# thevasudevgupta/gsoc-wav2vec2

Hardware: AMD Instinct MI355X
Metric: audio-seconds/s (wav2vec2-base forward, 246000-sample pad) (higher is better)
Workload: dtype f32

## Files before the change

gsoc-wav2vec2_amd/csrc/common.h:

```cpp
#pragma once

#include <hip/hip_runtime.h>
#include <stdint.h>
#include <stdio.h>

#include <atomic>

#include <string>

#include "../../include/w2v2.h"

namespace w2v2 {

void set_error(const char* fmt, ...);

#define W2V2_HIP_CHECK(expr)                                                            \
    do {                                                                                \
        hipError_t _e = (expr);                                                         \
        if (_e != hipSuccess) {                                                         \
            ::w2v2::set_error("%s failed: %s (%s:%d)", #expr, hipGetErrorString(_e),    \
                              __FILE__, __LINE__);                                      \
            return W2V2_EHIP;                                                           \
        }                                                                               \
    } while (0)
// ... 98 lines not shown
    ~ProfScope() {
        if (--tl_prof_depth == 0) tl_launch_family = outer_family;
        if (tok >= 0) profiler_end(p, tok, s);
    }
};

extern thread_local Profiler* tl_step_prof;
struct StepProfScope {
    Profiler* outer;
    explicit StepProfScope(Profiler* p) : outer(tl_step_prof) { tl_step_prof = p; }
    ~StepProfScope() { tl_step_prof = outer; }
};

int launch_gemm(Profiler* prof, const float* A, int64_t lda, int64_t strideA, const float* B,
                int64_t ldb, float* C, int64_t ldc, int64_t strideC, const float* bias,
                const float* residual, int M, int N, int K, int nbatch, int act, hipStream_t s);

void gemm_f32_force_ring(int route);
bool gemm_f32_ring_ok(int tile, const float* A, int64_t lda, int64_t strideA, const float* B, int64_t ldb, int64_t strideB,
                      int M, int N, int K);
int launch_gemm_f32_ring(int tile, bool persist, const float* A, int64_t lda, int64_t strideA, const float* B, int64_t ldb,
                         int64_t strideB, float* C, int64_t ldc, int64_t strideC, const float* bias, const float* residual, int M,
                         int N, int K, int nbatch, int act, hipStream_t s);
int launch_gemm_f32_ring_split(bool persist, int64_t main_tiles, const float* A, int64_t lda, const float* B, int64_t ldb, float* C,
                               int64_t ldc, const float* bias, const float* residual, int M, int N, int K, int act, hipStream_t s);

int launch_gemm_bf16(Profiler* prof, const float* A, int64_t lda, int64_t strideA, const float* B, int64_t ldb,
                     int64_t strideB, float* C, int64_t ldc, int64_t strideC, const float* bias,
                     const float* residual, int M, int N, int K, int nbatch, int act, hipStream_t s);
bool gemm_split_supported(const float* A, int64_t lda, int64_t strideA, int M, int N, int K);
int launch_split_weight(const float* w, uint16_t* planes, int K, int N, hipStream_t s);
int launch_gemm_split(Profiler* prof, const float* A, int64_t lda, int64_t strideA, const uint16_t* planes, float* C, int64_t ldc,
                      int64_t strideC, const float* bias, const float* residual, int M, int N, int K, int nbatch, int act,
                      hipStream_t s);

bool gemm_split_sw_ok(const uint16_t* A16, int64_t planeA, int64_t lda, int64_t strideA, int M, int N, int K);
int launch_split_weight_sw(const float* w, uint16_t* img, int K, int N, int fmt, void* scratch, hipStream_t s);
int launch_split_planes(const float* x, uint16_t* planes, int64_t plane, int64_t n, int fmt, int* range_flag, hipStream_t s);
int launch_gemm_split_sw(Profiler* prof, int fmt, const uint16_t* A16, int64_t planeA, int64_t lda, int64_t strideA, const uint16_t* Bimg,
                         const float* out_scale, float* C, uint16_t* C16, int64_t planeC, int64_t ldc, int64_t strideC, const float* bias,
                         const float* residual, int M, int N, int K, int nbatch, int act, int* range_flag, hipStream_t s);

int launch_check_select_forms(unsigned long long* mismatches_dev , hipStream_t s);

struct GemmShadows {
    const uint16_t* A16 = nullptr;
    const uint16_t* B16 = nullptr;
    uint16_t* C16 = nullptr;
// ... 345 lines not shown
```

gsoc-wav2vec2_amd/csrc/gemm_f32.hip:

```cpp
#include <stdlib.h>


#include "common.h"
#include "gemm_epilogue.h"

namespace w2v2 {

using f32x16 = __attribute__((ext_vector_type(16))) float;
using f32x4 = __attribute__((ext_vector_type(4))) float;

namespace {

constexpr int BK = 32;
constexpr int LDA_S = BK + 4;

struct GemmArgs {
    const float* A;
    const float* B;
    float* C;
    const float* bias;
    const float* residual;
    int64_t lda, ldb, ldc, strideA, strideB, strideC;
    int M, N, K, act;
    int tiles_m, tiles_n;
// ... 326 lines not shown
        const int64_t e = i * 4, row = e / N;
        const int col = (int)(e % N);
        float4 acc = reinterpret_cast<const float4*>(slabs)[i];
        for (int z = 1; z < S; ++z) {
            const float4 v = reinterpret_cast<const float4*>(slabs + (int64_t)z * M * N)[i];
            acc.x += v.x; acc.y += v.y; acc.z += v.z; acc.w += v.w;
        }
        if (bias) { acc.x += bias[col]; acc.y += bias[col + 1]; acc.z += bias[col + 2]; acc.w += bias[col + 3]; }
        acc.x = apply_act(acc.x, act); acc.y = apply_act(acc.y, act); acc.z = apply_act(acc.z, act); acc.w = apply_act(acc.w, act);
        if (residual) {
            const float4 r = *reinterpret_cast<const float4*>(residual + row * ldc + col);
            acc.x += r.x; acc.y += r.y; acc.z += r.z; acc.w += r.w;
        }
        *reinterpret_cast<float4*>(C + row * ldc + col) = acc;
    }
}

thread_local int tl_precision = 0;
thread_local int tl_ring = -1;

constexpr int RING_DEFAULT = 2;
int ring_route() { return tl_ring >= 0 ? tl_ring : tune_int("W2V2_GEMM_RING", RING_DEFAULT); }

}

void gemm_set_precision(int mode) { tl_precision = mode; }
void gemm_f32_force_ring(int route) { tl_ring = route; }
int gemm_get_precision() { return tl_precision; }

int launch_gemm(Profiler* prof, const float* A, int64_t lda, int64_t strideA, const float* B,
                int64_t ldb, float* C, int64_t ldc, int64_t strideC, const float* bias,
                const float* residual, int M, int N, int K, int nbatch, int act, hipStream_t s) {
    return launch_gemm_ex(prof, A, lda, strideA, B, ldb, 0, C, ldc, strideC, bias, residual, M, N, K, nbatch, act, s);
}

int launch_gemm_ex(Profiler* prof, const float* A, int64_t lda, int64_t strideA, const float* B,
                   int64_t ldb, int64_t strideB, float* C, int64_t ldc, int64_t strideC, const float* bias,
                   const float* residual, int M, int N, int K, int nbatch, int act, hipStream_t s) {
    if (tl_precision == 1)
        return launch_gemm_bf16(prof, A, lda, strideA, B, ldb, strideB, C, ldc, strideC, bias, residual, M, N, K, nbatch, act, s);
    W2V2_REQUIRE(A && B && C, "gemm: null operand");
    W2V2_REQUIRE(M > 0 && N > 0 && K > 0 && nbatch > 0, "gemm: bad sizes M=%d N=%d K=%d batch=%d", M, N, K, nbatch);
    W2V2_REQUIRE(lda >= 1 && ldb >= N && ldc >= N && ldc < (1 << 23), "gemm: bad leading dimensions");
    W2V2_REQUIRE(act >= 0 && act <= 2, "gemm: bad activation %d", act);
    GemmArgs g;
    g.A = A; g.B = B; g.C = C; g.bias = bias; g.residual = residual;
    g.lda = lda; g.ldb = ldb; g.ldc = ldc; g.strideA = strideA; g.strideB = strideB; g.strideC = strideC;
    g.M = M; g.N = N; g.K = K; g.act = act;
    const bool fast = (K % BK == 0) && (N % 4 == 0) && (lda % 4 == 0) && (ldb % 4 == 0) &&
                      (strideA % 4 == 0) && (strideB % 4 == 0) && ((reinterpret_cast<uintptr_t>(A) & 15) == 0) &&
                      ((reinterpret_cast<uintptr_t>(B) & 15) == 0);
    ProfScope ps(prof, FAM_GEMM, 2.0 * M * (double)N * K * nbatch,
                 4.0 * nbatch * ((double)M * K + (double)M * N) + 4.0 * (double)K * N, s);
    int cfg = forced_cfg();
    const bool by_shape = cfg < 0;
    if (cfg < 0 && fast && nbatch == 1 && strideB == 0 && K >= 1024 && (ldc % 4) == 0 &&
        ((reinterpret_cast<uintptr_t>(C) | reinterpret_cast<uintptr_t>(residual) | reinterpret_cast<uintptr_t>(bias)) & 15) == 0) {
        const int64_t tiles64 = (int64_t)((M + 63) / 64) * ((N + 63) / 64);
        int S = 1;
        for (int cand = 8; cand >= 2; cand >>= 1)
            if (K % (cand * BK) == 0 && K / cand >= 256 && tiles64 * cand <= 512) { S = cand; break; }
        if (S > 1 && tiles64 <= 256) {
            const size_t need = (size_t)S * M * N;
// ... 2 lines not shown
            if (int e = stream_scratch(SCRATCH_SPLITK, s, need * sizeof(float), &raw)) return e;
            ws = reinterpret_cast<float*>(raw);
            GemmArgs h = g;
            h.C = ws; h.bias = nullptr; h.residual = nullptr; h.act = 0;
            h.K = K / S; h.strideA = K / S; h.strideB = (int64_t)(K / S) * ldb; h.ldc = N; h.strideC = (int64_t)M * N;
            if (int e = launch_dma<2, 2, 2, 32, 64, 64>(h, S, s)) return e;
            const int64_t n4 = (int64_t)M * N / 4;
            int64_t blocks = (n4 + 255) / 256;
            blocks = blocks > 2048 ? 2048 : blocks;
            W2V2_LAUNCH(splitk_reduce_kernel, dim3((unsigned)blocks), dim3(256), 0, s, ws, C, bias, residual, M, N, ldc, S, act);
            W2V2_HIP_CHECK(hipGetLastError());
            return W2V2_OK;
        }
    }
    if (cfg < 0) {
        cfg = 7;
        const int64_t tiles128 = (int64_t)((M + 127) / 128) * ((N + 127) / 128) * nbatch;
        if (fast && tiles128 < 384) cfg = 16;
        const int tail_knob = tune_int("W2V2_GEMM_TAIL", 1);
        const int64_t tn = (N + 127) / 128, S = 512, r = tiles128 % S;
        if (tail_knob && fast && cfg == 7 && nbatch == 1 && tiles128 > S && r != 0 && tune_int("W2V2_GEMM_TAIL_DIV", 4) * r <= S) {
            const int64_t main_rows = ((tiles128 - r) / tn) * 128;
            const int ring_flat = by_shape && tune_int("W2V2_GEMM_TAIL_FLAT", 1) ? ring_route() : 0;
            if (ring_flat && strideB == 0 && M % 128 == 0 && N % 128 == 0 && gemm_f32_ring_ok(1, A, lda, 0, B, ldb, 0, M, N, K) &&
                gemm_f32_ring_ok(2, A, lda, 0, B, ldb, 0, M, N, K))
                return launch_gemm_f32_ring_split(ring_flat == 2, tiles128 - r, A, lda, B, ldb, C, ldc, bias, residual, M, N, K, act, s);
            if (main_rows > 0 && main_rows < M) {
                GemmArgs h = g;
                h.M = (int)main_rows;
                const int ring = by_shape ? ring_route() : 0;
                if (ring && strideB == 0 && gemm_f32_ring_ok(1, A, lda, strideA, B, ldb, strideB, h.M, N, K)) {
                    if (int e = launch_gemm_f32_ring(1, ring == 2, A, lda, strideA, B, ldb, strideB, C, ldc, strideC, bias, residual,
                                                     h.M, N, K, 1, act, s))
                        return e;
                } else if (int e = launch_dma<2, 4, 2>(h, 1, s)) {
                    return e;
                }
                GemmArgs t = g;
                t.A = g.A + main_rows * lda;
                t.C = g.C + main_rows * ldc;
                t.residual = g.residual ? g.residual + main_rows * ldc : nullptr;
                t.M = M - (int)main_rows;
                if (ring && strideB == 0 && gemm_f32_ring_ok(2, t.A, lda, strideA, B, ldb, strideB, t.M, N, K))
                    return launch_gemm_f32_ring(2, ring == 2, t.A, lda, strideA, B, ldb, strideB, t.C, ldc, strideC, bias,
                                                t.residual, t.M, N, K, 1, act, s);
                return launch_dma<2, 2, 2, 32, 64, 64>(t, 1, s);
            }
        }
    }
    if (cfg == 16 && fast && by_shape) {
        const int ring = ring_route();
        if (ring && strideB == 0 && gemm_f32_ring_ok(2, A, lda, strideA, B, ldb, strideB, M, N, K))
            return launch_gemm_f32_ring(2, ring == 2, A, lda, strideA, B, ldb, strideB, C, ldc, strideC, bias, residual, M, N, K,
                                        nbatch, act, s);
    }
    const int wide_min = tune_int("W2V2_GEMM_WIDE", 1536);
    if (cfg == 7 && fast && wide_min > 0 && N % 128 == 0) {
        const int64_t tm256 = (M + 255) / 256, tiles256 = tm256 * (N / 128) * nbatch;
        if (tiles256 >= wide_min && (tm256 * 256 - M) * 40 <= M) {
            const int ring = by_shape ? ring_route() : 0;
            if (ring && strideB == 0 && gemm_f32_ring_ok(0, A, lda, strideA, B, ldb, strideB, M, N, K))
                return launch_gemm_f32_ring(0, ring == 2, A, lda, strideA, B, ldb, strideB, C, ldc, strideC, bias, residual, M, N, K,
                                            nbatch, act, s);
            return launch_dma<4, 2, 2, 16, 256, 128>(g, nbatch, s);
        }
    }
    if (cfg == 7 && fast) {
        const int ring = by_shape ? ring_route() : 0;
        if (ring && strideB == 0 && gemm_f32_ring_ok(1, A, lda, strideA, B, ldb, strideB, M, N, K))
            return launch_gemm_f32_ring(1, ring == 2, A, lda, strideA, B, ldb, strideB, C, ldc, strideC, bias, residual, M, N, K,
                                        nbatch, act, s);
    }
    switch (cfg) {
        case 16: if (fast) return launch_dma<2, 2, 2, 32, 64, 64>(g, nbatch, s); return launch_cfg<128, 128, 2, 2, 2>(g, fast, nbatch, s);
        case 14: if (fast) return launch_dma<2, 3, 2, 32, 128, 96>(g, nbatch, s); return launch_cfg<128, 128, 2, 2, 2>(g, fast, nbatch, s);
        case 1: return launch_cfg<128, 256, 2, 2, 1>(g, fast, nbatch, s);
        case 2: return launch_cfg<256, 128, 2, 2, 1>(g, fast, nbatch, s);
        case 3: return launch_cfg<256, 256, 4, 2, 2>(g, fast, nbatch, s);
        case 4: if (fast) return launch_dma<2, 2, 2>(g, nbatch, s); return launch_cfg<128, 128, 2, 2, 2>(g, fast, nbatch, s);
        case 6: if (fast) return launch_dma<4, 2, 2>(g, nbatch, s); return launch_cfg<128, 128, 2, 2, 2>(g, fast, nbatch, s);
        case 7: if (fast) return launch_dma<2, 4, 2>(g, nbatch, s); return launch_cfg<128, 128, 2, 2, 2>(g, fast, nbatch, s);
        case 9: if (fast) return launch_dma<2, 4, 3, 16>(g, nbatch, s); return launch_cfg<128, 128, 2, 2, 2>(g, fast, nbatch, s);
        case 10: if (fast) return launch_dma<2, 4, 4, 16>(g, nbatch, s); return launch_cfg<128, 128, 2, 2, 2>(g, fast, nbatch, s);
        case 11: if (fast) return launch_dma<2, 2, 4, 16>(g, nbatch, s); return launch_cfg<128, 128, 2, 2, 2>(g, fast, nbatch, s);
        case 12: if (fast && g.N >= 256) return launch_dma<4, 4, 1, 32, 256, 256>(g, nbatch, s); return launch_cfg<128, 128, 2, 2, 2>(g, fast, nbatch, s);
        case 13: if (fast && g.N >= 128) return launch_dma<4, 2, 1, 32, 256, 128>(g, nbatch, s); return launch_cfg<128, 128, 2, 2, 2>(g, fast, nbatch, s);
        case 8: if (fast) return launch_dma<4, 4, 1>(g, nbatch, s); return launch_cfg<128, 128, 2, 2, 2>(g, fast, nbatch, s);
#ifdef W2V2_TUNING
        case 17: if (fast && g.N >= 256) return launch_dma<2, 4, 2, 16, 128, 256>(g, nbatch, s); return launch_dma<2, 4, 2>(g, nbatch, s);
        case 18: if (fast && g.N >= 128) return launch_dma<4, 2, 2, 16, 256, 128>(g, nbatch, s); return launch_dma<2, 4, 2>(g, nbatch, s);
        case 19: if (fast && g.N >= 256) return launch_dma<2, 4, 2, 32, 128, 256>(g, nbatch, s); return launch_dma<2, 4, 2>(g, nbatch, s);
#endif
        default: return launch_cfg<128, 128, 2, 2, 2>(g, fast, nbatch, s);
    }
// ... 4 lines not shown
```

gsoc-wav2vec2_amd/csrc/gemm_f32_sw.hip:

```cpp
#include "common.h"
#include "gemm_epilogue.h"
#include "gemm_sw_common.h"

namespace w2v2 {

namespace {

struct GemmRingArgs {
    const float* A;
    const float* B;
    float* C;
    const float* bias;
    const float* residual;
    int64_t lda, ldb, ldc, strideA, strideB, strideC;
    int M, N, K, act;
    int tiles_m, tiles_n, nbatch;
    int gm;
    int total;
    int first;
};

template <int WM, int WN, int BKT, int BM, int BN, int NS>
struct RingCfg {
    static constexpr int STAGE = (BM * BKT + BKT * BN) * 4;
    static constexpr int LDS = NS * STAGE;
    static constexpr int NW = WM * WN;
    static constexpr int NPA = BM * BKT / 256, NPB = BKT * BN / 256;
    static constexpr int PPA = NPA / NW, PPB = NPB / NW;
    static constexpr int P = PPA + PPB;
    static_assert(NPA % NW == 0 && NPB % NW == 0, "every wave issues the same number of pieces (counted waits)");
    static_assert((NS - 2) * P <= 63, "vmcnt field");
};

template <int WM, int WN, int BKT, int BM, int BN, int NS, bool QUAD = false>
__global__ __launch_bounds__(WM* WN * 64) __attribute__((amdgpu_waves_per_eu(4))) void gemm_f32_ring_kernel(GemmRingArgs g) {
    using R_ = RingCfg<WM, WN, BKT, BM, BN, NS>;
    constexpr int NW = R_::NW, PPA = R_::PPA, PPB = R_::PPB, P = R_::P, STAGE = R_::STAGE;
    constexpr int RPP = 256 / BKT;
    constexpr int SPR = BKT / 4;
    constexpr int SW = BKT == 32 ? 1 : 2;
    constexpr int WTM = BM / WM, WTN = BN / WN, MT = WTM / 32, NTL = WTN / 32;
    extern __shared__ __attribute__((aligned(16))) float smem[];
    const int tid = threadIdx.x, lane = tid & 63, wave = __builtin_amdgcn_readfirstlane(tid >> 6);
    const int wm = wave / WN, wn = wave % WN, li = lane & 31, lh = lane >> 5;
    const unsigned lds0 = (unsigned)(uintptr_t)(__attribute__((address_space(3))) float*)smem;

    const int nwg = g.tiles_m * g.tiles_n, total = g.total, G = gridDim.x;
    const int ntl = (total - (int)blockIdx.x + G - 1) / G;
    const int nk = g.K / BKT, nsteps = ntl * nk;
    auto tile_of = [&](int i, int& z, int& m0, int& n0) {
        const int v = (int)blockIdx.x + i * G;
        const int q = total >> 3, r = total & 7, xcd = v & 7, idx = v >> 3;
        int t = (xcd < r ? xcd * (q + 1) : r * (q + 1) + (xcd - r) * q) + idx;
        int sub = 0;
        if constexpr (QUAD) {
            sub = t & 3;
            t = g.first + (t >> 2);
        }
        z = t / nwg;
        t -= z * nwg;
        int tm = t / g.tiles_n, tn = t % g.tiles_n;
        if (g.gm > 0) grouped_tile(t, g.tiles_m, g.tiles_n, g.gm, tm, tn);
        m0 = tm * BM;
        n0 = tn * BN;
        if constexpr (QUAD) {
            m0 = 2 * m0 + (sub >> 1) * BM;
            n0 = 2 * n0 + (sub & 1) * BN;
        }
    };

    int ii = 0, ikt = 0, ist = 0;
    const unsigned char* baseA = nullptr;
    const unsigned char* baseB = nullptr;
    uint32_t offA[PPA], offB[PPB];
    auto uniform_ptr = [](const void* p) {
        const uint64_t v = reinterpret_cast<uint64_t>(p);
        const uint32_t lo = __builtin_amdgcn_readfirstlane((uint32_t)v), hi = __builtin_amdgcn_readfirstlane((uint32_t)(v >> 32));
        return reinterpret_cast<const unsigned char*>(((uint64_t)hi << 32) | lo);
    };
    auto set_issue_tile = [&](int i) {
        int z, m0, n0;
        tile_of(i, z, m0, n0);
        baseA = uniform_ptr(g.A + (int64_t)z * g.strideA + (int64_t)m0 * g.lda);
        baseB = uniform_ptr(g.B + (int64_t)z * g.strideB + n0);
#pragma unroll
        for (int p = 0; p < PPA; ++p) {
            const int r = (wave + p * NW) * RPP + lane / SPR;
            const int rr = m0 + r < g.M ? r : g.M - 1 - m0;
// ... 82 lines not shown
            const bool more = s + NS - 1 < nsteps;
            if (more) issue_step();
            __builtin_amdgcn_sched_barrier(0);
            compute(cst);
            __builtin_amdgcn_sched_barrier(0);
            ring_barrier(more);
            cst = cst + 1 == NS ? 0 : cst + 1;
        }
        int z, m0, n0;
        tile_of(ci, z, m0, n0);
        const int64_t tile_off = (int64_t)z * g.strideC + (int64_t)(m0 + wm * WTM) * g.ldc + (n0 + wn * WTN);
        int act = g.act, ldc = (int)g.ldc, eli = li, elh = lh;
        const float* res = g.residual;
        const float* bias = g.bias;
        asm volatile("" : "+s"(act), "+s"(res), "+s"(bias), "+s"(ldc), "+v"(eli), "+v"(elh));
        __builtin_amdgcn_s_setprio(0);
        gemm_epilogue<MT, NTL, false>(acc, g.C + tile_off, nullptr, res ? res + tile_off : nullptr, bias ? bias + (n0 + wn * WTN) : nullptr,
                                     ldc, g.M - (m0 + wm * WTM), g.N - (n0 + wn * WTN), act, eli, elh);
        __builtin_amdgcn_s_setprio(1);
    }
    __builtin_amdgcn_s_setprio(0);
}

template <int WM, int WN, int BKT, int BM, int BN, int NS, bool QUAD = false>
int launch_ring(GemmRingArgs& g, bool persist, hipStream_t s, int64_t first = -1, int gm = 0) {
    using R_ = RingCfg<WM, WN, BKT, BM, BN, NS>;
    static_assert(2 * R_::LDS <= 160 * 1024, "two blocks per CU");
    constexpr int TM = QUAD ? 2 * BM : BM, TN = QUAD ? 2 * BN : BN;
    g.tiles_m = (g.M + TM - 1) / TM;
    g.tiles_n = (g.N + TN - 1) / TN;
    int64_t total = (int64_t)g.tiles_m * g.tiles_n * g.nbatch;
    W2V2_REQUIRE(first < 0 || (first > 0 && first < total && g.nbatch == 1 && g.M % TM == 0 && g.N % TN == 0), "gemm ring: bad split");
    W2V2_REQUIRE(!QUAD || first > 0, "gemm ring: quarter tiles need a split");
    g.first = QUAD ? (int)first : 0;
    if (first > 0) total = QUAD ? 4 * (total - first) : first;
    W2V2_REQUIRE(total < (1ll << 31), "gemm ring: %lld tiles", (long long)total);
    g.total = (int)total;
    constexpr int PER_CU = WM * WN == 8 ? 2 : 160 * 1024 / R_::LDS > 4 ? 4 : 160 * 1024 / R_::LDS;
    int grid = (int)total;
    if (persist) {
        int dev = 0, cus = 0;
        W2V2_HIP_CHECK(hipGetDevice(&dev));
        W2V2_HIP_CHECK(hipDeviceGetAttribute(&cus, hipDeviceAttributeMultiprocessorCount, dev));
        const int resident = (PER_CU * cus) & ~7;
        if (resident >= 8 && total > resident) grid = resident;
    }
    g.gm = first > 0 ? gm : g.nbatch == 1 ? tile_group_rows(g.tiles_m, g.tiles_n, (int64_t)BM * g.K * 4, BM == 256 ? 96 : 32 * PER_CU) : 0;
    static std::atomic<bool> attr_set{false};
    if (!attr_set) {
        W2V2_HIP_CHECK(hipFuncSetAttribute(reinterpret_cast<const void*>(gemm_f32_ring_kernel<WM, WN, BKT, BM, BN, NS, QUAD>),
                                           hipFuncAttributeMaxDynamicSharedMemorySize, R_::LDS));
        attr_set = true;
    }
    W2V2_LAUNCH((gemm_f32_ring_kernel<WM, WN, BKT, BM, BN, NS, QUAD>), dim3(grid), dim3(WM * WN * 64), R_::LDS, s, g);
    W2V2_HIP_CHECK(hipGetLastError());
    return W2V2_OK;
}

}

bool gemm_f32_ring_ok(int tile, const float* A, int64_t lda, int64_t strideA, const float* B, int64_t ldb, int64_t strideB,
                      int M, int N, int K) {
    const int BM = tile == 0 ? 256 : tile == 1 ? 128 : 64, BKT = tile == 2 ? 32 : 16;
    const bool align = ((reinterpret_cast<uintptr_t>(A) | reinterpret_cast<uintptr_t>(B)) & 15) == 0 && lda % 4 == 0 &&
                       ldb % 4 == 0 && strideA % 4 == 0 && strideB % 4 == 0;
    return align && K % BKT == 0 && N % 4 == 0 && N >= 4 && (int64_t)BM * lda * 4 < (1ll << 31) &&
           (int64_t)BKT * ldb * 4 < (1ll << 31) && M > 0;
}

int launch_gemm_f32_ring(int tile, bool persist, const float* A, int64_t lda, int64_t strideA, const float* B, int64_t ldb,
                         int64_t strideB, float* C, int64_t ldc, int64_t strideC, const float* bias, const float* residual, int M,
                         int N, int K, int nbatch, int act, hipStream_t s) {
    W2V2_REQUIRE(tile >= 0 && tile <= 2, "gemm ring: tile %d", tile);
    W2V2_REQUIRE(gemm_f32_ring_ok(tile, A, lda, strideA, B, ldb, strideB, M, N, K), "gemm ring: unsupported shape M=%d N=%d K=%d", M, N, K);
    GemmRingArgs g;
    g.A = A; g.B = B; g.C = C; g.bias = bias; g.residual = residual;
    g.lda = lda; g.ldb = ldb; g.ldc = ldc; g.strideA = strideA; g.strideB = strideB; g.strideC = strideC;
    g.M = M; g.N = N; g.K = K; g.act = act; g.nbatch = nbatch;
    if (tile == 0) return launch_ring<4, 2, 16, 256, 128, 3>(g, persist, s);
    if (tile == 1) return launch_ring<2, 4, 16, 128, 128, 4>(g, persist, s);
    return launch_ring<2, 2, 32, 64, 64, 3>(g, persist, s);
}

int launch_gemm_f32_ring_split(bool persist, int64_t main_tiles, const float* A, int64_t lda, const float* B, int64_t ldb, float* C,
                               int64_t ldc, const float* bias, const float* residual, int M, int N, int K, int act, hipStream_t s) {
    W2V2_REQUIRE(M % 128 == 0 && N % 128 == 0 && gemm_f32_ring_ok(1, A, lda, 0, B, ldb, 0, M, N, K) && gemm_f32_ring_ok(2, A, lda, 0, B, ldb, 0, M, N, K),
                 "gemm ring split: unsupported shape M=%d N=%d K=%d", M, N, K);
    GemmRingArgs g;
    g.A = A; g.B = B; g.C = C; g.bias = bias; g.residual = residual;
    g.lda = lda; g.ldb = ldb; g.ldc = ldc; g.strideA = 0; g.strideB = 0; g.strideC = 0;
    g.M = M; g.N = N; g.K = K; g.act = act; g.nbatch = 1;
    const int gm = tile_group_rows(M / 128, N / 128, (int64_t)128 * K * 4, 64);
    if (int e = launch_ring<2, 4, 16, 128, 128, 4>(g, persist, s, main_tiles, gm)) return e;
    return launch_ring<2, 2, 32, 64, 64, 3, true>(g, false, s, main_tiles, gm);
}

}
```

gsoc-wav2vec2_amd/csrc/w2v2_api.hip:

```cpp
#include <algorithm>
#include <mutex>
#include <atomic>
#include <stdarg.h>
#include <stdlib.h>
#include <string.h>

#include <map>
#include <string>
#include <unordered_map>
#include <vector>

#include "common.h"
#include "model.h"

namespace w2v2 {

static thread_local char g_err[1024] = "";
void set_error(const char* fmt, ...) {
    va_list ap;
    va_start(ap, fmt);
    vsnprintf(g_err, sizeof(g_err), fmt, ap);
    va_end(ap);
}

// ... 597 lines not shown
}
int w2v2_profile_reset(w2v2_model* m) {
    W2V2_REQUIRE(m, "profile_reset: null model");
    profiler_reset(m->prof);
    return W2V2_OK;
}

int w2v2_op_gemm(const float* A, int64_t lda, int64_t strideA, const float* B, int64_t ldb, float* C,
                 int64_t ldc, int64_t strideC, const float* bias, const float* residual, int32_t M,
                 int32_t N, int32_t K, int32_t nbatch, int32_t act, void* stream) {
    return launch_gemm(nullptr, A, lda, strideA, B, ldb, C, ldc, strideC, bias, residual, M, N, K, nbatch, act,
                       reinterpret_cast<hipStream_t>(stream));
}
int w2v2_op_gemm_variant(const float* A, int64_t lda, int64_t strideA, const float* B, int64_t ldb, float* C,
                         int64_t ldc, int64_t strideC, const float* bias, const float* residual, int32_t M,
                         int32_t N, int32_t K, int32_t nbatch, int32_t act, int32_t variant, void* stream) {
    W2V2_REQUIRE(variant >= -1 && variant <= 2, "op_gemm_variant: variant %d (-1 by shape, 0 double buffer, 1 ring, 2 persistent ring)", variant);
    gemm_f32_force_ring(variant);
    const int e = launch_gemm(nullptr, A, lda, strideA, B, ldb, C, ldc, strideC, bias, residual, M, N, K, nbatch, act,
                              reinterpret_cast<hipStream_t>(stream));
    gemm_f32_force_ring(-1);
    return e;
}
int w2v2_op_set_precision(int32_t mode) {
    W2V2_REQUIRE(mode >= W2V2_PRECISION_FP32 && mode <= W2V2_PRECISION_F16X2, "op_set_precision: unknown mode %d", mode);
    gemm_set_precision(mode);
    return W2V2_OK;
}
int w2v2_op_gemm_bf16(const float* A, int64_t lda, int64_t strideA, const float* B, int64_t ldb, float* C,
                      int64_t ldc, int64_t strideC, const float* bias, const float* residual, int32_t M,
                      int32_t N, int32_t K, int32_t nbatch, int32_t act, void* stream) {
    return launch_gemm_bf16(nullptr, A, lda, strideA, B, ldb, 0, C, ldc, strideC, bias, residual, M, N, K, nbatch, act,
                            reinterpret_cast<hipStream_t>(stream));
}
int w2v2_op_gemm_bf16_shadows(const uint16_t* A16, int64_t lda, int64_t strideA, const uint16_t* B16, float* C, uint16_t* C16, int64_t ldc,
                              int64_t strideC, const float* bias, const float* residual, int32_t M, int32_t N, int32_t K, int32_t nbatch,
                              int32_t act, int32_t variant, void* stream) {
    W2V2_REQUIRE(A16 && B16 && (C || C16), "op_gemm_bf16_shadows: null operand");
    W2V2_REQUIRE(variant >= 0 && variant <= 2, "op_gemm_bf16_shadows: variant %d (0 by shape, 1 = 128 x 128 tiles, 2 = 128 x 256 software-pipelined)", variant);
    W2V2_REQUIRE(variant != 2 || gemm_bf16_sw_ok(M, N, K, lda, K, strideA),
                 "op_gemm_bf16_shadows: variant 2 needs N %% 256 == 0, K %% 64 == 0, K >= 192 and 16-byte aligned rows");
    GemmShadows x;
    x.A16 = A16; x.B16 = B16; x.C16 = C16; x.ldb16 = K; x.force_kernel = variant;
    return launch_gemm_bf16_x(nullptr, nullptr, lda, strideA, nullptr, N, 0, C, ldc, strideC, bias, residual, M, N, K, nbatch, act, x,
                              reinterpret_cast<hipStream_t>(stream));
}
// ... 164 lines not shown
```

gsoc-wav2vec2_amd/wav2vec2/_native.py:

```python

import ctypes as C
import os

_HERE = os.path.dirname(os.path.abspath(__file__))
_PKG_ROOT = os.path.dirname(_HERE)
LIB_PATH = os.path.join(_PKG_ROOT, "lib", "libw2v2.so")

MAX_CONV_LAYERS = 16
ALIGN_MAX_LABELS = 8191
BEAM_MAX_WIDTH = 64
BEAM_MAX_VOCAB = 64
CUTS_CHUNK = 1024
CUTS_MAX_FRAMES = 1 << 24
RESAMPLE_TILE = 2048
RESAMPLE_MAX_L = 4096
RESAMPLE_MAX_TABLE = 1 << 22
EDIT_MAX_LEN = 65535
WORDLM_MAX_ORDER = 5


class W2V2Config(C.Structure):
    _fields_ = [
        ("vocab_size", C.c_int32),
        ("hidden_size", C.c_int32),
# ... 91 lines not shown
    "w2v2_op_pos_conv_ex": (C.c_int, [_P, _P, _P, _P, _P, _P, _I32, _I32, _I32, _I32, _I32, _I32, _I32, _I32, _P]),
    "w2v2_op_pos_conv_bf16_pack_elems": (_I64, [_I32, _I32, _I32, _I32]),
    "w2v2_op_pos_conv_weight_shadow": (C.c_int, [_P, _P, _I32, _I32, _I32, _P]),
    "w2v2_op_pos_conv_bf16": (C.c_int, [_P, _P, _P, _P, _P, _P, _P, _P, _I32, _I32, _I32, _I32, _I32, _I32, _I32, _I32, _P]),
    "w2v2_op_pos_conv_flip_regroup": (C.c_int, [_P, _P, _I32, _I32, _I32, _P]),
    "w2v2_op_pos_conv_dw": (C.c_int, [_P, _P, _P, _I32, _I32, _I32, _I32, _I32, _P]),
    "w2v2_pos_conv_dw_bf16_ws_floats": (C.c_int, [_I32, _I32, _I32, _I32, _I32, C.POINTER(_I64), C.POINTER(_I32)]),
    "w2v2_op_pos_conv_dw_bf16": (C.c_int, [_P, _P, _P, _P, _P, _P, _P, _I32, _I32, _I32, _I32, _I32, _P]),
    "w2v2_op_weight_norm_bwd": (C.c_int, [_P, _P, _P, _P, _P, _I32, _I32, _I32, _I32, _P]),
    "w2v2_activation_info": (C.c_int, [_P, C.c_char_p, C.POINTER(_I64)]),
    "w2v2_copy_activation": (C.c_int, [_P, C.c_char_p, _P, _I64, _P]),
    "w2v2_profile_enable": (C.c_int, [_P, C.c_int]),
    "w2v2_profile_families": (C.c_int, [_P, C.c_uint32]),
    "w2v2_profile_sampling": (C.c_int, [_P, C.c_int32]),
    "w2v2_profile_seen": (C.c_int, [_P, C.c_int, C.POINTER(_I64)]),
    "w2v2_profile_kernel_launches": (C.c_int, [_P, C.c_int, C.POINTER(_I64)]),
    "w2v2_profile_num_families": (C.c_int, []),
    "w2v2_clock_probe": (C.c_int, [_P, _I32, _P, C.POINTER(_I32)]),
    "w2v2_profile_read": (C.c_int, [_P, C.c_int, C.POINTER(C.c_char_p), C.POINTER(_I64),
                                    C.POINTER(C.c_double), C.POINTER(C.c_double), C.POINTER(C.c_double)]),
    "w2v2_profile_reset": (C.c_int, [_P]),
    "w2v2_op_gemm": (C.c_int, [_P, _I64, _I64, _P, _I64, _P, _I64, _I64, _P, _P, _I32, _I32, _I32, _I32, _I32, _P]),
    "w2v2_op_gemm_variant": (C.c_int, [_P, _I64, _I64, _P, _I64, _P, _I64, _I64, _P, _P, _I32, _I32, _I32, _I32, _I32, _I32, _P]),
    "w2v2_op_set_precision": (C.c_int, [_I32]),
    "w2v2_op_gemm_split": (C.c_int, [_P, _I64, _I64, _P, _P, _I64, _I64, _P, _P, _I32, _I32, _I32, _I32, _I32, _P]),
    "w2v2_op_gemm_bf16_at": (C.c_int, [_P, _I64, _I64, _P, _I64, _I64, _P, _I64, _I64, _I32, _I32, _I32, _I32, _P]),
    "w2v2_crc32c_extend": (C.c_uint32, [C.c_uint32, _P, C.c_uint64]),
    "w2v2_op_weight_grad_bf16": (C.c_int, [_P, _P, _P, _I64, _I32, _I32, _I32, _I32, _I32, _P]),
    "w2v2_op_check_select_forms": (C.c_int, [_P, _P]),
    "w2v2_op_split_planes": (C.c_int, [_P, _P, _I64, _I64, _I32, _P, _P]),
    "w2v2_op_split_weight": (C.c_int, [_P, _P, _P, _I32, _I32, _I32, _P]),
    "w2v2_op_gemm_split_planes": (C.c_int, [_I32, _P, _I64, _I64, _I64, _P, _P, _P, _P, _I64, _I64, _I64, _P, _P, _I32, _I32, _I32, _I32, _I32, _P, _P]),
    "w2v2_op_gemm_bf16_shadows": (C.c_int, [_P, _I64, _I64, _P, _P, _P, _I64, _I64, _P, _P, _I32, _I32, _I32, _I32, _I32, _I32, _P]),
    "w2v2_op_gemm_bf16": (C.c_int, [_P, _I64, _I64, _P, _I64, _P, _I64, _I64, _P, _P, _I32, _I32, _I32, _I32, _I32, _P]),
    "w2v2_op_layer_norm": (C.c_int, [_P, _P, _P, _P, _I64, _I32, C.c_float, _I32, _P]),
    "w2v2_conv0_ws_floats": (_I64, [_I32, _I64, _I32, _I32, _I32]),
    "w2v2_op_conv0": (C.c_int, [_P, _P, _P, _P, _P, _P, _P, _I32, _I64, _I32, _I32, _I32, C.c_float, _I32, _I32, _P]),
    "w2v2_op_weight_norm_regroup": (C.c_int, [_P, _P, _P, _I32, _I32, _I32, _I32, _P]),
    "w2v2_op_pos_conv": (C.c_int, [_P, _P, _P, _P, _P, _I32, _I32, _I32, _I32, _I32, _I32, _P]),
    "w2v2_op_attention": (C.c_int, [_P, _P, _P, _I32, _I32, _I32, _I32, _P]),
    "w2v2_op_attention_packed": (C.c_int, [_P, _I32, _P, _P, _P, _I64, _P, _I32, _I32, _P]),
    "w2v2_op_frame_lengths": (C.c_int, [_P, _P, _I32, _I64, C.POINTER(_I32), C.POINTER(_I32), _I32, _P]),
    "w2v2_op_normalize_windows": (C.c_int, [_P, _I32, _P, _P, _P, _P]),
}

_lib = None
# ... 90 lines not shown
```

include/w2v2.h:

```cpp
#ifndef W2V2_H_
#define W2V2_H_

#include <stdint.h>

#ifdef __cplusplus
extern "C" {
#endif

#define W2V2_MAX_CONV_LAYERS 16

enum {
    W2V2_OK = 0,
    W2V2_EINVAL = -1,
    W2V2_ENOTFOUND = -2,
    W2V2_EHIP = -3,
    W2V2_ESTATE = -4
};

typedef struct w2v2_config {
    int32_t vocab_size;
    int32_t hidden_size;
    int32_t num_heads;
    int32_t num_layers;
    int32_t intermediate_size;
// ... 160 lines not shown
int w2v2_profile_enable(w2v2_model* m, int enable);
int w2v2_profile_families(w2v2_model* m, uint32_t family_mask);
int w2v2_profile_sampling(w2v2_model* m, int32_t stride);
int w2v2_profile_seen(w2v2_model* m, int index, int64_t* launches);
int w2v2_profile_kernel_launches(w2v2_model* m, int index, int64_t* launches);
int w2v2_profile_num_families(void);
int w2v2_profile_read(w2v2_model* m, int index, const char** name, int64_t* launches,
                      double* total_ms, double* flops, double* bytes);
int w2v2_profile_reset(w2v2_model* m);

int w2v2_clock_probe(void* stream, int32_t spin_us, uint64_t* dev_out4, int32_t* wall_clock_khz);


int w2v2_op_gemm(const float* A_dev, int64_t lda, int64_t strideA,
                 const float* B_dev, int64_t ldb,
                 float* C_dev, int64_t ldc, int64_t strideC,
                 const float* bias_dev, const float* residual_dev,
                 int32_t M, int32_t N, int32_t K, int32_t nbatch, int32_t act, void* stream);
int w2v2_op_gemm_variant(const float* A_dev, int64_t lda, int64_t strideA,
                         const float* B_dev, int64_t ldb,
                         float* C_dev, int64_t ldc, int64_t strideC,
                         const float* bias_dev, const float* residual_dev,
                         int32_t M, int32_t N, int32_t K, int32_t nbatch, int32_t act, int32_t variant, void* stream);

int w2v2_op_set_precision(int32_t mode);

int w2v2_op_gemm_bf16(const float* A_dev, int64_t lda, int64_t strideA,
                      const float* B_dev, int64_t ldb,
                      float* C_dev, int64_t ldc, int64_t strideC,
                      const float* bias_dev, const float* residual_dev,
                      int32_t M, int32_t N, int32_t K, int32_t nbatch, int32_t act, void* stream);

int w2v2_op_gemm_bf16_shadows(const uint16_t* A16_dev, int64_t lda, int64_t strideA, const uint16_t* B16_nk_dev, float* C_dev,
                              uint16_t* C16_dev, int64_t ldc, int64_t strideC, const float* bias_dev, const float* residual_dev,
                              int32_t M, int32_t N, int32_t K, int32_t nbatch, int32_t act, int32_t variant, void* stream);

int w2v2_op_gemm_split(const float* A_dev, int64_t lda, int64_t strideA, const float* B_dev,
                       float* C_dev, int64_t ldc, int64_t strideC,
                       const float* bias_dev, const float* residual_dev,
                       int32_t M, int32_t N, int32_t K, int32_t nbatch, int32_t act, void* stream);

#define W2V2_PLANES_BF16X3 0
#define W2V2_PLANES_F16X2 1
int w2v2_op_split_planes(const float* x_dev, uint16_t* planes_dev, int64_t plane_stride, int64_t n, int32_t fmt, int32_t* range_flag_dev,
                         void* stream);
int w2v2_op_split_weight(const float* B_dev, uint16_t* images_dev, float* scale_ws_dev, int32_t K, int32_t N, int32_t fmt, void* stream);
// ... 101 lines not shown
```

Baseline: 8365.

## Generalize ring GEMM tail split to ragged, 256-row and batched shapes

Extends the ring GEMM main/tail split so that full tiles run in the big-tile kernel and the leftover wave of tiles (including ragged M or N edges) runs as 64x64 pieces in a second launch. It now applies to the 256-row wide path and to ragged single-batch shapes by default, with batched and padded-wide variants behind knobs. The aim is to cut tail-wave underutilization and padded-tile waste. The cost is an extra kernel launch and more complex piece-index mapping. It also adds a launch log for introspection.

```diff
diff --git a/gsoc-wav2vec2_amd/csrc/common.h b/gsoc-wav2vec2_amd/csrc/common.h
--- a/gsoc-wav2vec2_amd/csrc/common.h
+++ b/gsoc-wav2vec2_amd/csrc/common.h
@@ -144,8 +144,11 @@
 int launch_gemm_f32_ring(int tile, bool persist, const float* A, int64_t lda, int64_t strideA, const float* B, int64_t ldb,
                          int64_t strideB, float* C, int64_t ldc, int64_t strideC, const float* bias, const float* residual, int M,
                          int N, int K, int nbatch, int act, hipStream_t s);
-int launch_gemm_f32_ring_split(bool persist, int64_t main_tiles, const float* A, int64_t lda, const float* B, int64_t ldb, float* C,
-                               int64_t ldc, const float* bias, const float* residual, int M, int N, int K, int act, hipStream_t s);
+int launch_gemm_f32_ring_split(int tile, bool persist, int64_t main_tiles, const float* A, int64_t lda, int64_t strideA, const float* B,
+                               int64_t ldb, float* C, int64_t ldc, int64_t strideC, const float* bias, const float* residual, int M, int N,
+                               int K, int nbatch, int act, hipStream_t s);
+void gemm_f32_ring_log_reset();
+int gemm_f32_ring_log(int32_t* records, int cap);
 
 int launch_gemm_bf16(Profiler* prof, const float* A, int64_t lda, int64_t strideA, const float* B, int64_t ldb,
                      int64_t strideB, float* C, int64_t ldc, int64_t strideC, const float* bias,
diff --git a/gsoc-wav2vec2_amd/csrc/gemm_f32.hip b/gsoc-wav2vec2_amd/csrc/gemm_f32.hip
--- a/gsoc-wav2vec2_amd/csrc/gemm_f32.hip
+++ b/gsoc-wav2vec2_amd/csrc/gemm_f32.hip
@@ -372,6 +372,19 @@
 constexpr int RING_DEFAULT = 2;
 int ring_route() { return tl_ring >= 0 ? tl_ring : tune_int("W2V2_GEMM_RING", RING_DEFAULT); }
 
+constexpr int SPLIT_RAGGED_DEFAULT = 1, SPLIT_BATCHED_DEFAULT = 0;
+constexpr int WIDE_SPLIT_DEFAULT = 0;
+int64_t ring_split_tiles(int tile, int M, int N, int nbatch) {
+    const int BM = tile == 0 ? 256 : 128;
+    const bool flat = tile == 1 && nbatch == 1 && M % 128 == 0 && N % 128 == 0;
+    if (!flat && tl_ring < 0 &&
+        !(nbatch > 1 ? tune_int("W2V2_GEMM_SPLIT_BATCHED", SPLIT_BATCHED_DEFAULT) : tune_int("W2V2_GEMM_SPLIT_RAGGED", SPLIT_RAGGED_DEFAULT)))
+        return 0;
+    const int64_t S = 512, whole = (int64_t)(M / BM) * ((N + 127) / 128) * nbatch, r = whole % S;
+    if (whole < S || tune_int("W2V2_GEMM_TAIL_DIV", 4) * r > S || (r == 0 && M % BM == 0)) return 0;
+    return whole - r;
+}
+
 }
 
 void gemm_set_precision(int mode) { tl_precision = mode; }
@@ -389,6 +402,7 @@
                    const float* residual, int M, int N, int K, int nbatch, int act, hipStream_t s) {
     if (tl_precision == 1)
         return launch_gemm_bf16(prof, A, lda, strideA, B, ldb, strideB, C, ldc, strideC, bias, residual, M, N, K, nbatch, act, s);
+    gemm_f32_ring_log_reset();
     W2V2_REQUIRE(A && B && C, "gemm: null operand");
     W2V2_REQUIRE(M > 0 && N > 0 && K > 0 && nbatch > 0, "gemm: bad sizes M=%d N=%d K=%d batch=%d", M, N, K, nbatch);
     W2V2_REQUIRE(lda >= 1 && ldb >= N && ldc >= N && ldc < (1 << 23), "gemm: bad leading dimensions");
@@ -437,9 +451,9 @@
         if (tail_knob && fast && cfg == 7 && nbatch == 1 && tiles128 > S && r != 0 && tune_int("W2V2_GEMM_TAIL_DIV", 4) * r <= S) {
             const int64_t main_rows = ((tiles128 - r) / tn) * 128;
             const int ring_flat = by_shape && tune_int("W2V2_GEMM_TAIL_FLAT", 1) ? ring_route() : 0;
-            if (ring_flat && strideB == 0 && M % 128 == 0 && N % 128 == 0 && gemm_f32_ring_ok(1, A, lda, 0, B, ldb, 0, M, N, K) &&
-                gemm_f32_ring_ok(2, A, lda, 0, B, ldb, 0, M, N, K))
-                return launch_gemm_f32_ring_split(ring_flat == 2, tiles128 - r, A, lda, B, ldb, C, ldc, bias, residual, M, N, K, act, s);
+            const int64_t main_tiles = ring_flat ? ring_split_tiles(1, M, N, 1) : 0;
+            if (main_tiles && strideB == 0 && gemm_f32_ring_ok(1, A, lda, 0, B, ldb, 0, M, N, K) && gemm_f32_ring_ok(2, A, lda, 0, B, ldb, 0, M, N, K))
+                return launch_gemm_f32_ring_split(1, ring_flat == 2, main_tiles, A, lda, 0, B, ldb, C, ldc, 0, bias, residual, M, N, K, 1, act, s);
             if (main_rows > 0 && main_rows < M) {
                 GemmArgs h = g;
                 h.M = (int)main_rows;
@@ -470,21 +484,33 @@
                                         nbatch, act, s);
     }
     const int wide_min = tune_int("W2V2_GEMM_WIDE", 1536);
+    const bool split_on = by_shape && tune_int("W2V2_GEMM_TAIL", 1) && tune_int("W2V2_GEMM_TAIL_FLAT", 1) && strideB == 0 && ring_route() != 0;
     if (cfg == 7 && fast && wide_min > 0 && N % 128 == 0) {
         const int64_t tm256 = (M + 255) / 256, tiles256 = tm256 * (N / 128) * nbatch;
-        if (tiles256 >= wide_min && (tm256 * 256 - M) * 40 <= M) {
+        const int64_t main_tiles = split_on ? ring_split_tiles(0, M, N, nbatch) : 0;
+        const bool padded_ok = (tm256 * 256 - M) * 40 <= M || (main_tiles != 0 && tune_int("W2V2_GEMM_WIDE_SPLIT", WIDE_SPLIT_DEFAULT) != 0);
+        if (tiles256 >= wide_min && padded_ok) {
             const int ring = by_shape ? ring_route() : 0;
-            if (ring && strideB == 0 && gemm_f32_ring_ok(0, A, lda, strideA, B, ldb, strideB, M, N, K))
+            if (ring && strideB == 0 && gemm_f32_ring_ok(0, A, lda, strideA, B, ldb, strideB, M, N, K)) {
+                if (main_tiles && gemm_f32_ring_ok(2, A, lda, strideA, B, ldb, strideB, M, N, K))
+                    return launch_gemm_f32_ring_split(0, ring == 2, main_tiles, A, lda, strideA, B, ldb, C, ldc, strideC, bias, residual, M, N, K,
+                                                      nbatch, act, s);
                 return launch_gemm_f32_ring(0, ring == 2, A, lda, strideA, B, ldb, strideB, C, ldc, strideC, bias, residual, M, N, K,
                                             nbatch, act, s);
+            }
             return launch_dma<4, 2, 2, 16, 256, 128>(g, nbatch, s);
         }
     }
     if (cfg == 7 && fast) {
         const int ring = by_shape ? ring_route() : 0;
-        if (ring && strideB == 0 && gemm_f32_ring_ok(1, A, lda, strideA, B, ldb, strideB, M, N, K))
+        if (ring && strideB == 0 && gemm_f32_ring_ok(1, A, lda, strideA, B, ldb, strideB, M, N, K)) {
+            const int64_t main_tiles = split_on ? ring_split_tiles(1, M, N, nbatch) : 0;
+            if (main_tiles && gemm_f32_ring_ok(2, A, lda, strideA, B, ldb, strideB, M, N, K))
+                return launch_gemm_f32_ring_split(1, ring == 2, main_tiles, A, lda, strideA, B, ldb, C, ldc, strideC, bias, residual, M, N, K,
+                                                  nbatch, act, s);
             return launch_gemm_f32_ring(1, ring == 2, A, lda, strideA, B, ldb, strideB, C, ldc, strideC, bias, residual, M, N, K,
                                         nbatch, act, s);
+        }
     }
     switch (cfg) {
         case 16: if (fast) return launch_dma<2, 2, 2, 32, 64, 64>(g, nbatch, s); return launch_cfg<128, 128, 2, 2, 2>(g, fast, nbatch, s);
diff --git a/gsoc-wav2vec2_amd/csrc/gemm_f32_sw.hip b/gsoc-wav2vec2_amd/csrc/gemm_f32_sw.hip
--- a/gsoc-wav2vec2_amd/csrc/gemm_f32_sw.hip
+++ b/gsoc-wav2vec2_amd/csrc/gemm_f32_sw.hip
@@ -18,6 +18,11 @@
     int gm;
     int total;
     int first;
+    int npa;
+    int sm;
+    int pnl;
+    int pme;
+    int off0;
 };
 
 template <int WM, int WN, int BKT, int BM, int BN, int NS>
@@ -32,7 +37,7 @@
     static_assert((NS - 2) * P <= 63, "vmcnt field");
 };
 
-template <int WM, int WN, int BKT, int BM, int BN, int NS, bool QUAD = false>
+template <int WM, int WN, int BKT, int BM, int BN, int NS, int PIECES = 0>
 __global__ __launch_bounds__(WM* WN * 64) __attribute__((amdgpu_waves_per_eu(4))) void gemm_f32_ring_kernel(GemmRingArgs g) {
     using R_ = RingCfg<WM, WN, BKT, BM, BN, NS>;
     constexpr int NW = R_::NW, PPA = R_::PPA, PPB = R_::PPB, P = R_::P, STAGE = R_::STAGE;
@@ -52,8 +57,43 @@
         const int v = (int)blockIdx.x + i * G;
         const int q = total >> 3, r = total & 7, xcd = v & 7, idx = v >> 3;
         int t = (xcd < r ? xcd * (q + 1) : r * (q + 1) + (xcd - r) * q) + idx;
+        if constexpr (PIECES == 2) {
+            static_assert(BM == 64 && BN == 64, "pieces are 64 x 64");
+            const int npc = 2 * g.tiles_n - (2 - g.pnl);
+            int tm, tn, sr, sc;
+            auto in_tile_row = [&](int rem, int pr) {
+                tn = rem / (2 * pr);
+                const int sub = rem - tn * 2 * pr, pn = tn == g.tiles_n - 1 ? g.pnl : 2;
+                sr = sub / pn;
+                sc = sub - sr * pn;
+            };
+            if (t >= g.npa) {
+                const int e = t - g.npa, per = g.pme * npc;
+                z = e / per;
+                tm = g.tiles_m;
+                in_tile_row(e - z * per, g.pme);
+            } else if (g.pnl == 2) {
+                const int per = 2 * g.sm;
+                int u = g.first + t / per;
+                const int sub = t % per;
+                z = u / nwg;
+                u -= z * nwg;
+                tm = u / g.tiles_n, tn = u % g.tiles_n;
+                if (g.gm > 0) grouped_tile(u, g.tiles_m, g.tiles_n, g.gm, tm, tn);
+                sr = sub >> 1;
+                sc = sub & 1;
+            } else {
+                const int p = g.off0 + t, per = g.sm * npc, row = p / per;
+                z = row / g.tiles_m;
+                tm = row - z * g.tiles_m;
+                in_tile_row(p - row * per, g.sm);
+            }
+            m0 = (tm * g.sm + sr) * 64;
+            n0 = (tn * 2 + sc) * 64;
+            return;
+        }
         int sub = 0;
-        if constexpr (QUAD) {
+        if constexpr (PIECES == 1) {
             sub = t & 3;
             t = g.first + (t >> 2);
         }
@@ -63,7 +103,7 @@
         if (g.gm > 0) grouped_tile(t, g.tiles_m, g.tiles_n, g.gm, tm, tn);
         m0 = tm * BM;
         n0 = tn * BN;
-        if constexpr (QUAD) {
+        if constexpr (PIECES == 1) {
             m0 = 2 * m0 + (sub >> 1) * BM;
             n0 = 2 * n0 + (sub & 1) * BN;
         }
@@ -192,39 +232,82 @@
     __builtin_amdgcn_s_setprio(0);
 }
 
-template <int WM, int WN, int BKT, int BM, int BN, int NS, bool QUAD = false>
-int launch_ring(GemmRingArgs& g, bool persist, hipStream_t s, int64_t first = -1, int gm = 0) {
+thread_local int tl_log_n = 0;
+thread_local int tl_log[4][4];
+void log_launch(int tile, int part, int total, int grid) {
+    if (tl_log_n < 4) {
+        int* r = tl_log[tl_log_n];
+        r[0] = tile; r[1] = part; r[2] = total; r[3] = grid;
+    }
+    ++tl_log_n;
+}
+
+template <int WM, int WN, int BKT, int BM, int BN, int NS, int PIECES = 0>
+int launch_ring_order(GemmRingArgs& g, bool persist, int part, hipStream_t s) {
     using R_ = RingCfg<WM, WN, BKT, BM, BN, NS>;
     static_assert(2 * R_::LDS <= 160 * 1024, "two blocks per CU");
-    constexpr int TM = QUAD ? 2 * BM : BM, TN = QUAD ? 2 * BN : BN;
-    g.tiles_m = (g.M + TM - 1) / TM;
-    g.tiles_n = (g.N + TN - 1) / TN;
-    int64_t total = (int64_t)g.tiles_m * g.tiles_n * g.nbatch;
-    W2V2_REQUIRE(first < 0 || (first > 0 && first < total && g.nbatch == 1 && g.M % TM == 0 && g.N % TN == 0), "gemm ring: bad split");
-    W2V2_REQUIRE(!QUAD || first > 0, "gemm ring: quarter tiles need a split");
-    g.first = QUAD ? (int)first : 0;
-    if (first > 0) total = QUAD ? 4 * (total - first) : first;
-    W2V2_REQUIRE(total < (1ll << 31), "gemm ring: %lld tiles", (long long)total);
-    g.total = (int)total;
     constexpr int PER_CU = WM * WN == 8 ? 2 : 160 * 1024 / R_::LDS > 4 ? 4 : 160 * 1024 / R_::LDS;
-    int grid = (int)total;
+    int grid = g.total;
     if (persist) {
         int dev = 0, cus = 0;
         W2V2_HIP_CHECK(hipGetDevice(&dev));
         W2V2_HIP_CHECK(hipDeviceGetAttribute(&cus, hipDeviceAttributeMultiprocessorCount, dev));
         const int resident = (PER_CU * cus) & ~7;
-        if (resident >= 8 && total > resident) grid = resident;
-    }
-    g.gm = first > 0 ? gm : g.nbatch == 1 ? tile_group_rows(g.tiles_m, g.tiles_n, (int64_t)BM * g.K * 4, BM == 256 ? 96 : 32 * PER_CU) : 0;
+        if (resident >= 8 && g.total > resident) grid = resident;
+    }
     static std::atomic<bool> attr_set{false};
     if (!attr_set) {
-        W2V2_HIP_CHECK(hipFuncSetAttribute(reinterpret_cast<const void*>(gemm_f32_ring_kernel<WM, WN, BKT, BM, BN, NS, QUAD>),
+        W2V2_HIP_CHECK(hipFuncSetAttribute(reinterpret_cast<const void*>(gemm_f32_ring_kernel<WM, WN, BKT, BM, BN, NS, PIECES>),
                                            hipFuncAttributeMaxDynamicSharedMemorySize, R_::LDS));
         attr_set = true;
     }
-    W2V2_LAUNCH((gemm_f32_ring_kernel<WM, WN, BKT, BM, BN, NS, QUAD>), dim3(grid), dim3(WM * WN * 64), R_::LDS, s, g);
+    log_launch(BM == 256 ? 0 : BM == 128 ? 1 : 2, part, g.total, grid);
+    W2V2_LAUNCH((gemm_f32_ring_kernel<WM, WN, BKT, BM, BN, NS, PIECES>), dim3(grid), dim3(WM * WN * 64), R_::LDS, s, g);
     W2V2_HIP_CHECK(hipGetLastError());
     return W2V2_OK;
+}
+
+inline int ring_group_rows(int BM, int tiles_m, int tiles_n, int K) {
+    return tile_group_rows(tiles_m, tiles_n, (int64_t)BM * K * 4, BM == 256 ? 96 : 64);
+}
+
+template <int WM, int WN, int BKT, int BM, int BN, int NS>
+int launch_ring(GemmRingArgs& g, bool persist, hipStream_t s) {
+    g.tiles_m = (g.M + BM - 1) / BM;
+    g.tiles_n = (g.N + BN - 1) / BN;
+    const int64_t total = (int64_t)g.tiles_m * g.tiles_n * g.nbatch;
+    W2V2_REQUIRE(total < (1ll << 31), "gemm ring: %lld tiles", (long long)total);
+    g.total = (int)total;
+    g.gm = g.nbatch == 1 ? ring_group_rows(BM, g.tiles_m, g.tiles_n, g.K) : 0;
+    g.first = 0;
+    return launch_ring_order<WM, WN, BKT, BM, BN, NS>(g, persist, 0, s);
+}
+
+template <int WM, int WN, int BM, int NS>
+int launch_ring_split(GemmRingArgs& g, bool persist, int64_t main_tiles, hipStream_t s) {
+    constexpr int SM = BM / 64;
+    const int tmf = g.M / BM, tn = (g.N + 127) / 128;
+    const int64_t nint = (int64_t)tmf * tn * g.nbatch;
+    W2V2_REQUIRE(main_tiles > 0 && main_tiles <= nint && (main_tiles < nint || g.M % BM), "gemm ring: bad split");
+    g.tiles_m = tmf;
+    g.tiles_n = tn;
+    g.sm = SM;
+    g.pnl = (g.N - (tn - 1) * 128 + 63) / 64;
+    g.pme = (g.M - tmf * BM + 63) / 64;
+    g.gm = g.nbatch == 1 && g.pnl == 2 ? ring_group_rows(BM, tmf, tn, g.K) : 0;
+    const int npc = 2 * tn - (2 - g.pnl);
+    auto before = [&](int64_t t) { return SM * (2 * t - (2 - g.pnl) * (t / tn)); };
+    const int64_t npa = before(nint) - before(main_tiles), pieces = npa + (int64_t)g.pme * npc * g.nbatch;
+    W2V2_REQUIRE(before(nint) + pieces < (1ll << 31), "gemm ring: %lld tiles", (long long)nint);
+    g.first = 0;
+    g.total = (int)main_tiles;
+    if (int e = launch_ring_order<WM, WN, 16, BM, 128, NS>(g, persist, 1, s)) return e;
+    g.first = (int)main_tiles;
+    g.off0 = (int)before(main_tiles);
+    g.npa = (int)npa;
+    g.total = (int)pieces;
+    if (SM == 2 && g.pme == 0 && g.pnl == 2 && g.nbatch == 1) return launch_ring_order<2, 2, 32, 64, 64, 3, 1>(g, false, 2, s);
+    return launch_ring_order<2, 2, 32, 64, 64, 3, 2>(g, false, 2, s);
 }
 
 }
@@ -252,17 +335,25 @@
     return launch_ring<2, 2, 32, 64, 64, 3>(g, persist, s);
 }
 
-int launch_gemm_f32_ring_split(bool persist, int64_t main_tiles, const float* A, int64_t lda, const float* B, int64_t ldb, float* C,
-                               int64_t ldc, const float* bias, const float* residual, int M, int N, int K, int act, hipStream_t s) {
-    W2V2_REQUIRE(M % 128 == 0 && N % 128 == 0 && gemm_f32_ring_ok(1, A, lda, 0, B, ldb, 0, M, N, K) && gemm_f32_ring_ok(2, A, lda, 0, B, ldb, 0, M, N, K),
+int launch_gemm_f32_ring_split(int tile, bool persist, int64_t main_tiles, const float* A, int64_t lda, int64_t strideA, const float* B,
+                               int64_t ldb, float* C, int64_t ldc, int64_t strideC, const float* bias, const float* residual, int M, int N,
+                               int K, int nbatch, int act, hipStream_t s) {
+    W2V2_REQUIRE((tile == 0 || tile == 1) && gemm_f32_ring_ok(tile, A, lda, strideA, B, ldb, 0, M, N, K) &&
+                     gemm_f32_ring_ok(2, A, lda, strideA, B, ldb, 0, M, N, K),
                  "gemm ring split: unsupported shape M=%d N=%d K=%d", M, N, K);
     GemmRingArgs g;
     g.A = A; g.B = B; g.C = C; g.bias = bias; g.residual = residual;
-    g.lda = lda; g.ldb = ldb; g.ldc = ldc; g.strideA = 0; g.strideB = 0; g.strideC = 0;
-    g.M = M; g.N = N; g.K = K; g.act = act; g.nbatch = 1;
-    const int gm = tile_group_rows(M / 128, N / 128, (int64_t)128 * K * 4, 64);
-    if (int e = launch_ring<2, 4, 16, 128, 128, 4>(g, persist, s, main_tiles, gm)) return e;
-    return launch_ring<2, 2, 32, 64, 64, 3, true>(g, false, s, main_tiles, gm);
-}
-
-}
+    g.lda = lda; g.ldb = ldb; g.ldc = ldc; g.strideA = strideA; g.strideB = 0; g.strideC = strideC;
+    g.M = M; g.N = N; g.K = K; g.act = act; g.nbatch = nbatch;
+    if (tile == 0) return launch_ring_split<4, 2, 256, 3>(g, persist, main_tiles, s);
+    return launch_ring_split<2, 4, 128, 4>(g, persist, main_tiles, s);
+}
+
+void gemm_f32_ring_log_reset() { tl_log_n = 0; }
+int gemm_f32_ring_log(int32_t* records, int cap) {
+    for (int i = 0; i < tl_log_n && i < 4 && i < cap; ++i)
+        for (int j = 0; j < 4; ++j) records[4 * i + j] = tl_log[i][j];
+    return tl_log_n;
+}
+
+}
diff --git a/gsoc-wav2vec2_amd/csrc/w2v2_api.hip b/gsoc-wav2vec2_amd/csrc/w2v2_api.hip
--- a/gsoc-wav2vec2_amd/csrc/w2v2_api.hip
+++ b/gsoc-wav2vec2_amd/csrc/w2v2_api.hip
@@ -643,6 +643,11 @@
     gemm_f32_force_ring(-1);
     return e;
 }
+int w2v2_op_gemm_launch_log(int32_t* records, int32_t cap, int32_t* count) {
+    W2V2_REQUIRE(records && count && cap >= 0, "op_gemm_launch_log: bad argument");
+    *count = gemm_f32_ring_log(records, cap);
+    return W2V2_OK;
+}
 int w2v2_op_set_precision(int32_t mode) {
     W2V2_REQUIRE(mode >= W2V2_PRECISION_FP32 && mode <= W2V2_PRECISION_F16X2, "op_set_precision: unknown mode %d", mode);
     gemm_set_precision(mode);
diff --git a/gsoc-wav2vec2_amd/wav2vec2/_native.py b/gsoc-wav2vec2_amd/wav2vec2/_native.py
--- a/gsoc-wav2vec2_amd/wav2vec2/_native.py
+++ b/gsoc-wav2vec2_amd/wav2vec2/_native.py
@@ -137,6 +137,7 @@
     "w2v2_profile_reset": (C.c_int, [_P]),
     "w2v2_op_gemm": (C.c_int, [_P, _I64, _I64, _P, _I64, _P, _I64, _I64, _P, _P, _I32, _I32, _I32, _I32, _I32, _P]),
     "w2v2_op_gemm_variant": (C.c_int, [_P, _I64, _I64, _P, _I64, _P, _I64, _I64, _P, _P, _I32, _I32, _I32, _I32, _I32, _I32, _P]),
+    "w2v2_op_gemm_launch_log": (C.c_int, [_P, _I32, _P]),
     "w2v2_op_set_precision": (C.c_int, [_I32]),
     "w2v2_op_gemm_split": (C.c_int, [_P, _I64, _I64, _P, _P, _I64, _I64, _P, _P, _I32, _I32, _I32, _I32, _I32, _P]),
     "w2v2_op_gemm_bf16_at": (C.c_int, [_P, _I64, _I64, _P, _I64, _I64, _P, _I64, _I64, _I32, _I32, _I32, _I32, _P]),
diff --git a/include/w2v2.h b/include/w2v2.h
--- a/include/w2v2.h
+++ b/include/w2v2.h
@@ -206,6 +206,7 @@
                          float* C_dev, int64_t ldc, int64_t strideC,
                          const float* bias_dev, const float* residual_dev,
                          int32_t M, int32_t N, int32_t K, int32_t nbatch, int32_t act, int32_t variant, void* stream);
+int w2v2_op_gemm_launch_log(int32_t* records, int32_t cap, int32_t* count);
 
 int w2v2_op_set_precision(int32_t mode);
 
```

New measurement: 8370, median of 2. About the same (+0.1%).
